# yeyupiaoling/MASR

Measured on NVIDIA H100. Metric: audio_seconds_per_second, higher is better.
Workload: dtype f32 (GEMMs: fp16x2-split operands on wgmma, fp32 accumulate; fp32-grade results)

## Files before the change

masr_b200/csrc/tc_common.cuh:

```cuda
#pragma once
#include <cuda.h>
#include <cuda_fp16.h>
#include <mutex>

#include "common.cuh"

namespace masr {

constexpr float kLoScale = 2048.0f, kLoInv = 1.0f / 2048.0f;

__device__ __forceinline__ uint32_t smem_u32(const void* p) { return (uint32_t)__cvta_generic_to_shared(p); }

__device__ __forceinline__ void mbar_init(uint64_t* bar, uint32_t count) {
    asm volatile("mbarrier.init.shared::cta.b64 [%0], %1;" ::"r"(smem_u32(bar)), "r"(count));
}
__device__ __forceinline__ void mbar_expect_tx(uint64_t* bar, uint32_t bytes) {
    asm volatile("mbarrier.arrive.expect_tx.shared::cta.b64 _, [%0], %1;" ::"r"(smem_u32(bar)), "r"(bytes) : "memory");
}
__device__ __forceinline__ void mbar_wait(uint64_t* bar, uint32_t parity) {
    asm volatile(
        "{\n\t"
        ".reg .pred P1;\n\t"
        "WAIT_LOOP:\n\t"
        "mbarrier.try_wait.parity.shared::cta.b64 P1, [%0], %1;\n\t"
        "@P1 bra DONE;\n\t"
        "bra WAIT_LOOP;\n\t"
        "DONE:\n\t"
        "}" ::"r"(smem_u32(bar)), "r"(parity) : "memory");
}
__device__ __forceinline__ void tma_load_2d(const CUtensorMap* map, uint64_t* bar, void* smem_dst, int c0, int c1) {
    asm volatile(
        "cp.async.bulk.tensor.2d.shared::cluster.global.mbarrier::complete_tx::bytes [%0], [%1, {%3, %4}], [%2];"
        ::"r"(smem_u32(smem_dst)), "l"(map), "r"(smem_u32(bar)), "r"(c0), "r"(c1) : "memory");
}
__device__ __forceinline__ void tma_load_2d_multicast(const CUtensorMap* map, uint64_t* bar, void* smem_dst, int c0, int c1,
                                                      uint16_t cta_mask) {
    asm volatile(
        "cp.async.bulk.tensor.2d.shared::cluster.global.mbarrier::complete_tx::bytes.multicast::cluster"
        " [%0], [%1, {%3, %4}], [%2], %5;"
        ::"r"(smem_u32(smem_dst)), "l"(map), "r"(smem_u32(bar)), "r"(c0), "r"(c1), "h"(cta_mask) : "memory");
}
__device__ __forceinline__ uint32_t cluster_map(uint32_t a, uint32_t rank) {
    uint32_t r;
    asm volatile("mapa.shared::cluster.u32 %0, %1, %2;" : "=r"(r) : "r"(a), "r"(rank));
    return r;
}
__device__ __forceinline__ void cluster_sync() {
    asm volatile("barrier.cluster.arrive.release.aligned;\n\tbarrier.cluster.wait.acquire.aligned;" ::: "memory");
}
__device__ __forceinline__ void tma_prefetch_desc(const CUtensorMap* map) {
    asm volatile("prefetch.tensormap [%0];" ::"l"(map) : "memory");
}
__device__ __forceinline__ bool elect_one_sync() {
    uint32_t pred = 0, laneid = 0;
    asm volatile(
        "{\n\t"
        ".reg .b32 %%rx;\n\t"
        ".reg .pred %%px;\n\t"
        "elect.sync %%rx|%%px, %2;\n\t"
        "@%%px mov.s32 %1, 1;\n\t"
        "mov.s32 %0, %%rx;\n\t"
        "}"
        : "+r"(laneid), "+r"(pred)
        : "r"(0xFFFFFFFFu));
    return pred != 0;
}

__device__ __forceinline__ void wgmma_fence() { asm volatile("wgmma.fence.sync.aligned;" ::: "memory"); }
__device__ __forceinline__ void wgmma_commit() { asm volatile("wgmma.commit_group.sync.aligned;" ::: "memory"); }
template <int N>
__device__ __forceinline__ void wgmma_wait() { asm volatile("wgmma.wait_group.sync.aligned %0;" ::"n"(N) : "memory"); }
template <int R>
__device__ __forceinline__ void reg_fence(float (&d)[R]) {
#pragma unroll
    for (int i = 0; i < R; ++i) asm volatile("" : "+f"(d[i])::"memory");
}
__device__ __forceinline__ void wgmma_m64n128k16_ss(float (&d)[64], uint64_t da, uint64_t db, uint32_t scale_d) {
    asm volatile(
        "{\n\t"
        ".reg .pred p;\n\t"
        "setp.ne.b32 p, %66, 0;\n\t"
        "wgmma.mma_async.sync.aligned.m64n128k16.f32.f16.f16 "
        "{%0, %1, %2, %3, %4, %5, %6, %7, %8, %9, %10, %11, %12, %13, %14, %15, "
        "%16, %17, %18, %19, %20, %21, %22, %23, %24, %25, %26, %27, %28, %29, %30, %31, "
        "%32, %33, %34, %35, %36, %37, %38, %39, %40, %41, %42, %43, %44, %45, %46, %47, "
        "%48, %49, %50, %51, %52, %53, %54, %55, %56, %57, %58, %59, %60, %61, %62, %63}, %64, %65, p, 1, 1, 0, 0;\n\t"
        "}"
        : "+f"(d[0]), "+f"(d[1]), "+f"(d[2]), "+f"(d[3]), "+f"(d[4]), "+f"(d[5]), "+f"(d[6]), "+f"(d[7]), "+f"(d[8]),
          "+f"(d[9]), "+f"(d[10]), "+f"(d[11]), "+f"(d[12]), "+f"(d[13]), "+f"(d[14]), "+f"(d[15]), "+f"(d[16]),
          "+f"(d[17]), "+f"(d[18]), "+f"(d[19]), "+f"(d[20]), "+f"(d[21]), "+f"(d[22]), "+f"(d[23]), "+f"(d[24]),
          "+f"(d[25]), "+f"(d[26]), "+f"(d[27]), "+f"(d[28]), "+f"(d[29]), "+f"(d[30]), "+f"(d[31]), "+f"(d[32]),
          "+f"(d[33]), "+f"(d[34]), "+f"(d[35]), "+f"(d[36]), "+f"(d[37]), "+f"(d[38]), "+f"(d[39]), "+f"(d[40]),
          "+f"(d[41]), "+f"(d[42]), "+f"(d[43]), "+f"(d[44]), "+f"(d[45]), "+f"(d[46]), "+f"(d[47]), "+f"(d[48]),
          "+f"(d[49]), "+f"(d[50]), "+f"(d[51]), "+f"(d[52]), "+f"(d[53]), "+f"(d[54]), "+f"(d[55]), "+f"(d[56]),
          "+f"(d[57]), "+f"(d[58]), "+f"(d[59]), "+f"(d[60]), "+f"(d[61]), "+f"(d[62]), "+f"(d[63])
        : "l"(da), "l"(db), "r"(scale_d));
}
template <int R>
__device__ __forceinline__ void setmaxnreg_inc() { asm volatile("setmaxnreg.inc.sync.aligned.u32 %0;" ::"n"(R)); }
template <int R>
__device__ __forceinline__ void setmaxnreg_dec() { asm volatile("setmaxnreg.dec.sync.aligned.u32 %0;" ::"n"(R)); }

__device__ __forceinline__ uint64_t gmma_desc_sw64(uint32_t smem_addr) {
    uint64_t d = 0;
    d |= (uint64_t)((smem_addr & 0x3FFFF) >> 4);
    d |= (uint64_t)1 << 16;
    d |= (uint64_t)(512 >> 4) << 32;
    d |= (uint64_t)2 << 62;
    return d;
}

__device__ __forceinline__ void add2(float& d0, float& d1, float a0, float a1, float b0, float b1) { d0 = a0 + b0; d1 = a1 + b1; }
__device__ __forceinline__ void sub2(float& d0, float& d1, float a0, float a1, float b0, float b1) { d0 = a0 - b0; d1 = a1 - b1; }
__device__ __forceinline__ void mul2(float& d0, float& d1, float a0, float a1, float b0, float b1) { d0 = a0 * b0; d1 = a1 * b1; }
__device__ __forceinline__ void split_f16(float x, __half& h, __half& l) {
    h = __float2half_rn(x);
    l = __float2half_rn((x - __half2float(h)) * kLoScale);
}
__device__ __forceinline__ void split_f16x2(float x0, float x1, __half2& h, __half2& l) {
    h = __floats2half2_rn(x0, x1);
    const float2 hf = __half22float2(h);
    float d0, d1;
    sub2(d0, d1, x0, x1, hf.x, hf.y);
    mul2(d0, d1, d0, d1, kLoScale, kLoScale);
    l = __floats2half2_rn(d0, d1);
}

__device__ __forceinline__ void mbar_arrive(uint64_t* bar) {
    asm volatile("mbarrier.arrive.shared::cta.b64 _, [%0];" ::"r"(smem_u32(bar)) : "memory");
}
__device__ __forceinline__ void mbar_arrive_cluster(uint32_t a, uint32_t pred) {
    asm volatile("{\n\t.reg .pred p;\n\tsetp.ne.u32 p, %1, 0;\n\t@p mbarrier.arrive.shared::cluster.b64 _, [%0];\n\t}"
                 ::"r"(a), "r"(pred) : "memory");
}

__device__ __forceinline__ void sts128(uint32_t a, const uint4& v) {
    asm volatile("st.shared.v4.b32 [%0], {%1, %2, %3, %4};" ::"r"(a), "r"(v.x), "r"(v.y), "r"(v.z), "r"(v.w) : "memory");
}
__device__ __forceinline__ uint4 lds128(uint32_t a) {
    uint4 v;
    asm volatile("ld.shared.v4.b32 {%0, %1, %2, %3}, [%4];" : "=r"(v.x), "=r"(v.y), "=r"(v.z), "=r"(v.w) : "r"(a) : "memory");
    return v;
}

typedef CUresult (*EncodeTiledFn)(CUtensorMap*, CUtensorMapDataType, cuuint32_t, void*, const cuuint64_t*, const cuuint64_t*,
                                  const cuuint32_t*, const cuuint32_t*, CUtensorMapInterleave, CUtensorMapSwizzle,
                                  CUtensorMapL2promotion, CUtensorMapFloatOOBfill);

inline EncodeTiledFn get_encode_fn() {
    static EncodeTiledFn fn = nullptr;
    static std::once_flag once;
    std::call_once(once, [] {
        void* p = nullptr;
        cudaDriverEntryPointQueryResult qres;
        if (cudaGetDriverEntryPoint("cuTensorMapEncodeTiled", &p, cudaEnableDefault, &qres) == cudaSuccess &&
            qres == cudaDriverEntryPointSuccess)
            fn = reinterpret_cast<EncodeTiledFn>(p);
    });
    return fn;
}

}
```

masr_b200/csrc/tc_gemm.cu:

```cuda
#include <cuda.h>
#include <cuda_fp16.h>
#include <math.h>
#include <mutex>
#include <stdlib.h>
#include <string.h>

#include "tc_common.cuh"

namespace masr {

constexpr int TBM = 128, TBN = 128, TBK = 32;
constexpr int TILE_BYTES = TBM * TBK * 2;
constexpr int STAGE_BYTES = 4 * TILE_BYTES;
constexpr int EW = 8;
constexpr int kStages = 5;
constexpr int RES_BYTES = TBM * TBN * 4;
constexpr int TC_THREADS = 32 * EW + 128;
constexpr int PRODUCER_REGS = 40, CONSUMER_REGS = 232;
static_assert(PRODUCER_REGS * 128 + CONSUMER_REGS * 32 * EW <= 65536, "register file of the SM");

struct TcParams {
    const float* bias;
    const float* residual;
    float* C;
    __half* Ch;
    __half* Cl;
    int64_t ldr, ldc;
    int M, N, K;
    int epi;
    float alpha;
    int conv_T2;
    int flags;
    float* part_m;
    float* part_s;
    int* part_i;
};

constexpr int EPI_CTC_PARTIAL = 8;

struct TcMaps {
    CUtensorMap a[8];
    CUtensorMap w[2];
};

constexpr int CHUNK_KB = 256 / TBK;
constexpr int CONV_TR = 6, CONV_W2 = 19, CONV_ROWS = CONV_TR * CONV_W2;

__device__ __forceinline__ void tma_load_4d(const CUtensorMap* map, uint64_t* bar, void* smem_dst, int c0, int c1, int c2, int c3) {
    asm volatile(
        "cp.async.bulk.tensor.4d.shared::cluster.global.mbarrier::complete_tx::bytes [%0], [%1, {%3, %4, %5, %6}], [%2];"
        ::"r"(smem_u32(smem_dst)), "l"(map), "r"(smem_u32(bar)), "r"(c0), "r"(c1), "r"(c2), "r"(c3) : "memory");
}

struct EpiCtx {
    uint32_t sb;
    int lane;
    int64_t row0;
    int nvalid;
};

template <int CH>
__device__ __forceinline__ void staged_store(const EpiCtx& c, const uint4 (&regs)[CH], uint8_t* g0, int64_t pitch_bytes) {
    constexpr int RSH = (CH == 8) ? 0 : (CH == 4) ? 1 : 2;
    constexpr int RPI = 32 / CH;
    __syncwarp();
#pragma unroll
    for (int k = 0; k < CH; ++k) sts128(c.sb + c.lane * (CH * 16) + ((k ^ ((c.lane >> RSH) & (CH - 1))) << 4), regs[k]);
    __syncwarp();
    const int sub = c.lane / CH, k = c.lane % CH;
    uint4 v[CH];
#pragma unroll
    for (int i = 0; i < CH; ++i) {
        const int row = i * RPI + sub;
        v[i] = lds128(c.sb + row * (CH * 16) + ((k ^ ((row >> RSH) & (CH - 1))) << 4));
    }
#pragma unroll
    for (int i = 0; i < CH; ++i) {
        const int row = i * RPI + sub;
        if (row < c.nvalid) *reinterpret_cast<uint4*>(g0 + row * pitch_bytes + (k << 4)) = v[i];
    }
}

__device__ __forceinline__ void staged_load(const EpiCtx& c, uint4 (&regs)[8], const uint8_t* g0, int64_t pitch_bytes) {
    __syncwarp();
    const int sub = c.lane >> 3, k = c.lane & 7;
    uint4 v[8];
#pragma unroll
    for (int i = 0; i < 8; ++i) {
        const int row = i * 4 + sub;
        v[i] = make_uint4(0, 0, 0, 0);
        if (row < c.nvalid) v[i] = *reinterpret_cast<const uint4*>(g0 + row * pitch_bytes + (k << 4));
    }
#pragma unroll
    for (int i = 0; i < 8; ++i) {
        const int row = i * 4 + sub;
        sts128(c.sb + row * 128 + ((k ^ (row & 7)) << 4), v[i]);
    }
    __syncwarp();
#pragma unroll
    for (int k2 = 0; k2 < 8; ++k2) regs[k2] = lds128(c.sb + c.lane * 128 + ((k2 ^ (c.lane & 7)) << 4));
}

template <int W, int STG>
__device__ __forceinline__ void emit_f32(const EpiCtx& c, float* C, int64_t ld, int flags, const float (&o)[W], int n, int n_limit) {
    const bool full = n + W - 1 < n_limit;
    const bool row_ok = c.lane < c.nvalid;
    const int64_t my_row = c.row0 + c.lane;
    if ((flags & 1) && full && (ld & 3) == 0 && (reinterpret_cast<uintptr_t>(C) & 15) == 0) {
        constexpr int CH = (W / 4 < STG / 512) ? W / 4 : STG / 512;
#pragma unroll
        for (int part = 0; part < (W / 4) / CH; ++part) {
            uint4 regs[CH];
#pragma unroll
            for (int j = 0; j < CH; ++j) {
                const int e = (part * CH + j) * 4;
                regs[j] = make_uint4(__float_as_uint(o[e]), __float_as_uint(o[e + 1]), __float_as_uint(o[e + 2]), __float_as_uint(o[e + 3]));
            }
            staged_store<CH>(c, regs, reinterpret_cast<uint8_t*>(C + c.row0 * ld + n + part * CH * 4), ld * 4);
        }
    } else if (row_ok && full && (ld & 3) == 0 && (reinterpret_cast<uintptr_t>(C) & 15) == 0) {
        float* cp = C + my_row * ld + n;
#pragma unroll
        for (int j = 0; j < W; j += 4) *reinterpret_cast<float4*>(cp + j) = make_float4(o[j], o[j + 1], o[j + 2], o[j + 3]);
    } else if (row_ok) {
        float* cp = C + my_row * ld + n;
#pragma unroll
        for (int j = 0; j < W; ++j)
            if (n + j < n_limit) cp[j] = o[j];
    }
}

template <int W, int STG>
__device__ __forceinline__ void emit_pair(const EpiCtx& c, __half* Ch, __half* Cl, int64_t ld, int flags, const float (&o)[W], int n,
                                          int n_limit) {
    const bool full = n + W - 1 < n_limit;
    const bool row_ok = c.lane < c.nvalid;
    const int64_t my_row = c.row0 + c.lane;
    uint32_t hh[W / 2], ll[W / 2];
#pragma unroll
    for (int j = 0; j < W / 2; ++j) {
        __half2 h2, l2;
        split_f16x2(o[2 * j], o[2 * j + 1], h2, l2);
        hh[j] = *reinterpret_cast<uint32_t*>(&h2);
        ll[j] = *reinterpret_cast<uint32_t*>(&l2);
    }
    const bool aligned = (ld & 7) == 0 && ((reinterpret_cast<uintptr_t>(Ch) | reinterpret_cast<uintptr_t>(Cl)) & 15) == 0;
    if ((flags & 1) && full && aligned) {
        constexpr int CH = (W / 8 < STG / 512) ? W / 8 : STG / 512;
#pragma unroll
        for (int part = 0; part < (W / 8) / CH; ++part) {
            uint4 regs[CH];
#pragma unroll
            for (int j = 0; j < CH; ++j) { const int e = 4 * (part * CH + j); regs[j] = make_uint4(hh[e], hh[e + 1], hh[e + 2], hh[e + 3]); }
            staged_store<CH>(c, regs, reinterpret_cast<uint8_t*>(Ch + c.row0 * ld + n + part * CH * 8), ld * 2);
#pragma unroll
            for (int j = 0; j < CH; ++j) { const int e = 4 * (part * CH + j); regs[j] = make_uint4(ll[e], ll[e + 1], ll[e + 2], ll[e + 3]); }
            staged_store<CH>(c, regs, reinterpret_cast<uint8_t*>(Cl + c.row0 * ld + n + part * CH * 8), ld * 2);
        }
    } else if (row_ok && full && aligned) {
        uint4* hp = reinterpret_cast<uint4*>(Ch + my_row * ld + n);
        uint4* lp = reinterpret_cast<uint4*>(Cl + my_row * ld + n);
#pragma unroll
        for (int j = 0; j < W / 8; ++j) {
            hp[j] = make_uint4(hh[4 * j], hh[4 * j + 1], hh[4 * j + 2], hh[4 * j + 3]);
            lp[j] = make_uint4(ll[4 * j], ll[4 * j + 1], ll[4 * j + 2], ll[4 * j + 3]);
        }
    } else if (row_ok) {
        unsigned short* hp = reinterpret_cast<unsigned short*>(Ch + my_row * ld + n);
        unsigned short* lp = reinterpret_cast<unsigned short*>(Cl + my_row * ld + n);
#pragma unroll
        for (int j = 0; j < W / 2; ++j) {
            if (n + 2 * j < n_limit) { hp[2 * j] = (unsigned short)(hh[j] & 0xffff); lp[2 * j] = (unsigned short)(ll[j] & 0xffff); }
            if (n + 2 * j + 1 < n_limit) { hp[2 * j + 1] = (unsigned short)(hh[j] >> 16); lp[2 * j + 1] = (unsigned short)(ll[j] >> 16); }
        }
    }
}

template <int W, int STG>
__device__ __forceinline__ void emit(const TcParams& p, const EpiCtx& c, const float (&o)[W], int n, int n_limit) {
    if (p.C) emit_f32<W, STG>(c, p.C, p.ldc, p.flags, o, n, n_limit);
    if (p.Ch) emit_pair<W, STG>(c, p.Ch, p.Cl, p.ldc, p.flags, o, n, n_limit);
}

template <int STG>
__device__ __forceinline__ void store_chunk(const TcParams& p, const EpiCtx& c, float (&v)[32], int n) {
    constexpr bool BIG = STG >= 4096;
    if (p.epi == EPI_CTC_PARTIAL) {
        if (n + 31 >= p.N) {
#pragma unroll
            for (int j = 0; j < 32; ++j)
                if (n + j >= p.N) v[j] = -INFINITY;
        }
        float m = v[0];
#pragma unroll
        for (int j = 1; j < 32; ++j) m = fmaxf(m, v[j]);
        int mj = 31;
#pragma unroll
        for (int j = 30; j >= 0; --j)
            if (v[j] == m) mj = j;
        const int mi = n + mj;
        const float mneg = -m * 1.4426950408889634f;
        float sum = 0.f;
#pragma unroll
        for (int j = 0; j < 32; ++j) sum += ex2_approx(fmaf(v[j], 1.4426950408889634f, mneg));
        if (c.lane < c.nvalid) {
            const int64_t idx = (int64_t)(n >> 5) * p.M + c.row0 + c.lane;
            p.part_m[idx] = m; p.part_s[idx] = sum; p.part_i[idx] = mi;
        }
        return;
    }
    if (p.epi == MASR_EPI_BIAS_GLU) {
        float o[16];
#pragma unroll
        for (int j = 0; j < 16; j += 8) {
            float e[8];
#pragma unroll
            for (int k = 0; k < 8; ++k) e[k] = ex2_approx(v[2 * (j + k) + 1] * -1.4426950408889634f);
#pragma unroll
            for (int k = 0; k < 8; ++k) e[k] = rcp_approx(1.0f + e[k]);
#pragma unroll
            for (int k = 0; k < 8; ++k) o[j + k] = v[2 * (j + k)] * e[k];
        }
        emit<16, STG>(p, c, o, n >> 1, p.N >> 1);
        return;
    }
    switch (p.epi) {
        case MASR_EPI_BIAS_SILU:
#pragma unroll
            for (int j = 0; j < 32; j += 8) {
                float e[8];
#pragma unroll
                for (int k = 0; k < 8; k += 2) mul2(e[k], e[k + 1], v[j + k], v[j + k + 1], -1.4426950408889634f, -1.4426950408889634f);
#pragma unroll
                for (int k = 0; k < 8; ++k) e[k] = ex2_approx(e[k]);
#pragma unroll
                for (int k = 0; k < 8; k += 2) add2(e[k], e[k + 1], e[k], e[k + 1], 1.0f, 1.0f);
#pragma unroll
                for (int k = 0; k < 8; ++k) e[k] = rcp_approx(e[k]);
#pragma unroll
                for (int k = 0; k < 8; k += 2) mul2(v[j + k], v[j + k + 1], v[j + k], v[j + k + 1], e[k], e[k + 1]);
            }
            break;
        case MASR_EPI_BIAS_RELU:
#pragma unroll
            for (int j = 0; j < 32; ++j) v[j] = v[j] != v[j] ? v[j] : fmaxf(v[j], 0.f);
            break;
        case MASR_EPI_BIAS_SCALE:
#pragma unroll
            for (int j = 0; j < 32; ++j) v[j] *= p.alpha;
            break;
        case MASR_EPI_RESIDUAL: {
            const bool vec_r = (p.ldr & 3) == 0 && (reinterpret_cast<uintptr_t>(p.residual) & 15) == 0;
            if (BIG && (p.flags & 2) && n + 31 < p.N && vec_r) {
                uint4 rr[8];
                staged_load(c, rr, reinterpret_cast<const uint8_t*>(p.residual + c.row0 * p.ldr + n), p.ldr * 4);
#pragma unroll
                for (int j = 0; j < 8; ++j) {
                    v[4 * j] = __uint_as_float(rr[j].x) + p.alpha * v[4 * j];
                    v[4 * j + 1] = __uint_as_float(rr[j].y) + p.alpha * v[4 * j + 1];
                    v[4 * j + 2] = __uint_as_float(rr[j].z) + p.alpha * v[4 * j + 2];
                    v[4 * j + 3] = __uint_as_float(rr[j].w) + p.alpha * v[4 * j + 3];
                }
            } else if (c.lane < c.nvalid && n + 31 < p.N && vec_r) {
                const float* r = p.residual + (c.row0 + c.lane) * p.ldr + n;
#pragma unroll
                for (int j = 0; j < 32; j += 4) {
                    const float4 rv = *reinterpret_cast<const float4*>(r + j);
                    v[j] = rv.x + p.alpha * v[j]; v[j + 1] = rv.y + p.alpha * v[j + 1];
                    v[j + 2] = rv.z + p.alpha * v[j + 2]; v[j + 3] = rv.w + p.alpha * v[j + 3];
                }
            } else if (c.lane < c.nvalid) {
                const float* r = p.residual + (c.row0 + c.lane) * p.ldr + n;
#pragma unroll
                for (int j = 0; j < 32; ++j)
                    if (n + j < p.N) v[j] = r[j] + p.alpha * v[j];
            }
            break;
        }
        default: break;
    }
    emit<32, STG>(p, c, v, n, p.N);
}

constexpr int EPI_STG = 4096;

__device__ __forceinline__ uint32_t res_off(int r, int c) { return (uint32_t)(r * 128 + ((((c >> 2) ^ (r & 7))) << 4) + (c & 3) * 4); }

template <bool CONV>
__global__ void __launch_bounds__(TC_THREADS, 1)
tc_gemm_kernel(const __grid_constant__ TcMaps maps, const __grid_constant__ TcParams p, int num_tiles, int tiles_n, int tiles_t) {
    extern __shared__ uint8_t smem_raw[];
    uint8_t* smem = reinterpret_cast<uint8_t*>((reinterpret_cast<uintptr_t>(smem_raw) + 1023) & ~uintptr_t(1023));
    uint8_t* res = smem + kStages * STAGE_BYTES;
    uint64_t* full_bar = reinterpret_cast<uint64_t*>(res + RES_BYTES);
    uint64_t* empty_bar = full_bar + kStages;

    const int warp = threadIdx.x >> 5, lane = threadIdx.x & 31;
    const int nkb = p.K / TBK;

    if (warp == EW && lane == 0) {
        tma_prefetch_desc(&maps.a[0]); tma_prefetch_desc(&maps.a[1]); tma_prefetch_desc(&maps.w[0]); tma_prefetch_desc(&maps.w[1]);
        for (int s = 0; s < kStages; ++s) { mbar_init(&full_bar[s], 1); mbar_init(&empty_bar[s], EW); }
        asm volatile("fence.mbarrier_init.release.cluster;" ::: "memory");
    }
    __syncthreads();
    pdl_wait();
    pdl_launch_dependents();

    auto decode = [&](int tile, int& n0, int& m0, int& t0, int& b) {
        const int nt = tile % tiles_n;
        const int rest = tile / tiles_n;
        n0 = nt * TBN;
        if (CONV) { t0 = (rest % tiles_t) * CONV_TR; b = rest / tiles_t; m0 = 0; }
        else { m0 = rest * TBM; t0 = 0; b = 0; }
    };

    if (warp >= EW) {
        setmaxnreg_dec<PRODUCER_REGS>();
        if (warp == EW && elect_one_sync()) {
            constexpr uint32_t a_bytes = CONV ? CONV_ROWS * TBK * 2 : TILE_BYTES;
            constexpr uint32_t tx_bytes = 2 * a_bytes + 2 * TILE_BYTES;
            uint32_t kg = 0;
            const int kb_tap = CONV ? p.N / TBK : 1;
            for (int tile = blockIdx.x; tile < num_tiles; tile += gridDim.x) {
                int n0, m0, t0, b;
                decode(tile, n0, m0, t0, b);
                for (int kb = 0; kb < nkb; ++kb, ++kg) {
                    const uint32_t s = kg % kStages;
                    mbar_wait(&empty_bar[s], ((kg / kStages) & 1) ^ 1);
                    uint8_t* st = smem + s * STAGE_BYTES;
                    if (p.flags & 32) {
                        mbar_arrive(&full_bar[s]);
                        continue;
                    }
                    mbar_expect_tx(&full_bar[s], tx_bytes);
                    if (CONV) {
                        const int tap = kb / kb_tap, cj = kb - tap * kb_tap;
                        const int kh = tap / 3, kw = tap - kh * 3;
                        const int plane = (kh & 1) * 2 + (kw & 1);
                        tma_load_4d(&maps.a[2 * plane], &full_bar[s], st, cj * TBK, kw >> 1, t0 + (kh >> 1), b);
                        tma_load_4d(&maps.a[2 * plane + 1], &full_bar[s], st + TILE_BYTES, cj * TBK, kw >> 1, t0 + (kh >> 1), b);
                    } else {
                        tma_load_2d(&maps.a[0], &full_bar[s], st, kb * TBK, m0);
                        tma_load_2d(&maps.a[1], &full_bar[s], st + TILE_BYTES, kb * TBK, m0);
                    }
                    tma_load_2d(&maps.w[0], &full_bar[s], st + 2 * TILE_BYTES, kb * TBK, n0);
                    tma_load_2d(&maps.w[1], &full_bar[s], st + 3 * TILE_BYTES, kb * TBK, n0);
                }
            }
        }
        __syncwarp();
    } else {
        setmaxnreg_inc<CONSUMER_REGS>();
        const int wg = warp >> 2, wi = warp & 3;
        uint8_t* wg_res = res + wg * (RES_BYTES / 2);
        const int nchunks = (nkb + CHUNK_KB - 1) / CHUNK_KB;
        EpiCtx ctx;
        ctx.lane = lane;
        auto map_rows = [&](int m0, int t0, int b, int q) {
            if (CONV) {
                const int rows = min(CONV_ROWS, (p.conv_T2 - t0) * CONV_W2);
                ctx.row0 = ((int64_t)b * p.conv_T2 + t0) * CONV_W2 + q * 32;
                ctx.nvalid = max(0, min(32, rows - q * 32));
            } else {
                ctx.row0 = (int64_t)m0 + q * 32;
                ctx.nvalid = max(0, min(32, p.M - (m0 + q * 32)));
            }
        };
        const uint32_t wg_bar = 1 + wg;
        const uint32_t is_lane0 = lane == 0;
        auto release = [&](uint32_t s) {
            asm volatile("{\n\t.reg .pred p;\n\tsetp.ne.u32 p, %1, 0;\n\t@p mbarrier.arrive.shared::cta.b64 _, [%0];\n\t}"
                         ::"r"(smem_u32(&empty_bar[s])), "r"(is_lane0) : "memory");
        };
        uint32_t kg = 0;
        for (int tile = blockIdx.x; tile < num_tiles; tile += gridDim.x) {
            int n0, m0, t0, b;
            decode(tile, n0, m0, t0, b);
            const int nw = n0 + wi * 32;
            if (p.bias != nullptr && nw + lane < p.N) asm volatile("prefetch.global.L1 [%0];" ::"l"(p.bias + nw + lane));
            float acc[64], cor[64];
            auto frag_addr = [&](int i, int hh) {
                const int R = 16 * wi + (lane >> 2) + 8 * hh, C = 8 * i + 2 * (lane & 3);
                return smem_u32(wg_res) + ((R >> 5) * 4 + (C >> 5)) * EPI_STG + res_off(R & 31, C & 31);
            };
            asm volatile("bar.sync %0, 128;" ::"r"(wg_bar) : "memory");
            if (p.flags & 64) {
                for (int kb = 0; kb < nkb; ++kb, ++kg) {
                    const uint32_t s = kg % kStages;
                    mbar_wait(&full_bar[s], (kg / kStages) & 1);
                    release(s);
                }
            } else for (int c = 0; c < nchunks; ++c) {
                const int kb_end = min(nkb, (c + 1) * CHUNK_KB);
                int pend = -1;
                for (int kb = c * CHUNK_KB; kb < kb_end; ++kb, ++kg) {
                    const uint32_t s = kg % kStages;
                    mbar_wait(&full_bar[s], (kg / kStages) & 1);
                    const uint32_t sa = smem_u32(smem + s * STAGE_BYTES);
                    const uint32_t sa_m = sa + wg * (TILE_BYTES / 2), sw = sa + 2 * TILE_BYTES;
                    const uint64_t dAh = gmma_desc_sw64(sa_m), dAl = gmma_desc_sw64(sa_m + TILE_BYTES);
                    const uint64_t dWh = gmma_desc_sw64(sw), dWl = gmma_desc_sw64(sw + TILE_BYTES);
                    reg_fence(acc); reg_fence(cor);
                    wgmma_fence();
#pragma unroll
                    for (int ks = 0; ks < TBK / 16; ++ks) {
                        const uint64_t adv = (uint64_t)(ks * 2);
                        wgmma_m64n128k16_ss(acc, dAh + adv, dWh + adv, (kb == c * CHUNK_KB && ks == 0) ? 0u : 1u);
                        wgmma_m64n128k16_ss(cor, dAh + adv, dWl + adv, (kb | ks) ? 1u : 0u);
                        wgmma_m64n128k16_ss(cor, dAl + adv, dWh + adv, 1u);
                    }
                    wgmma_commit();
                    wgmma_wait<1>();
                    reg_fence(acc); reg_fence(cor);
                    if (pend >= 0) release((uint32_t)pend);
                    pend = (int)s;
                }
                wgmma_wait<0>();
                reg_fence(acc); reg_fence(cor);
                if (pend >= 0) release((uint32_t)pend);
                if (c + 1 < nchunks) {
#pragma unroll
                    for (int i = 0; i < 16; ++i)
#pragma unroll
                        for (int hh = 0; hh < 2; ++hh) {
                            float x0 = acc[4 * i + 2 * hh], x1 = acc[4 * i + 2 * hh + 1];
                            const uint32_t a = frag_addr(i, hh);
                            if (c > 0) {
                                float s0, s1;
                                asm volatile("ld.shared.v2.f32 {%0, %1}, [%2];" : "=f"(s0), "=f"(s1) : "r"(a) : "memory");
                                x0 = s0 + x0; x1 = s1 + x1;
                            }
                            asm volatile("st.shared.v2.f32 [%0], {%1, %2};" ::"r"(a), "f"(x0), "f"(x1) : "memory");
                        }
                }
            }
#pragma unroll
            for (int i = 0; i < 16; ++i)
#pragma unroll
                for (int hh = 0; hh < 2; ++hh) {
                    const uint32_t a = frag_addr(i, hh);
                    float x0 = acc[4 * i + 2 * hh], x1 = acc[4 * i + 2 * hh + 1];
                    if (nchunks > 1) {
                        float s0, s1;
                        asm volatile("ld.shared.v2.f32 {%0, %1}, [%2];" : "=f"(s0), "=f"(s1) : "r"(a) : "memory");
                        x0 = s0 + x0; x1 = s1 + x1;
                    }
                    x0 = fmaf(cor[4 * i + 2 * hh], kLoInv, x0);
                    x1 = fmaf(cor[4 * i + 2 * hh + 1], kLoInv, x1);
                    asm volatile("st.shared.v2.f32 [%0], {%1, %2};" ::"r"(a), "f"(x0), "f"(x1) : "memory");
                }
            asm volatile("bar.sync %0, 128;" ::"r"(wg_bar) : "memory");
            for (int h = 0; h < 2; ++h) {
                const int q = 2 * wg + h;
                map_rows(m0, t0, b, q);
                ctx.sb = smem_u32(wg_res) + (h * 4 + wi) * EPI_STG;
                if (nw >= p.N) continue;
                float v[32];
#pragma unroll
                for (int k = 0; k < 8; ++k) {
                    const uint4 r4 = lds128(ctx.sb + lane * 128 + ((k ^ (lane & 7)) << 4));
                    v[4 * k] = __uint_as_float(r4.x); v[4 * k + 1] = __uint_as_float(r4.y);
                    v[4 * k + 2] = __uint_as_float(r4.z); v[4 * k + 3] = __uint_as_float(r4.w);
                }
                if (p.bias != nullptr && nw + 31 < p.N && (reinterpret_cast<uintptr_t>(p.bias + nw) & 15) == 0) {
#pragma unroll
                    for (int j = 0; j < 32; j += 4) {
                        const float4 bb = ldg_f4(p.bias + nw + j);
                        v[j] += bb.x; v[j + 1] += bb.y; v[j + 2] += bb.z; v[j + 3] += bb.w;
                    }
                } else if (p.bias != nullptr) {
#pragma unroll
                    for (int j = 0; j < 32; ++j)
                        if (nw + j < p.N) v[j] += __ldg(p.bias + nw + j);
                }
                store_chunk<EPI_STG>(p, ctx, v, nw);
            }
        }
    }
    __syncthreads();
}

constexpr size_t kTcSmem = kStages * STAGE_BYTES + RES_BYTES + 1024 + 256;
static_assert(kTcSmem <= 232448, "tc_gemm shared memory exceeds the 227 KB per-CTA limit of sm_90");

__global__ void __launch_bounds__(256) split_f16_kernel(const float* __restrict__ x, __half* __restrict__ h,
                                                        __half* __restrict__ l, int64_t n) {
    int64_t i = ((int64_t)blockIdx.x * 256 + threadIdx.x) * 4;
    if (i + 3 < n) {
        float4 v = ldg_f4(x + i);
        __half hh[4], ll[4];
        split_f16(v.x, hh[0], ll[0]); split_f16(v.y, hh[1], ll[1]); split_f16(v.z, hh[2], ll[2]); split_f16(v.w, hh[3], ll[3]);
        *reinterpret_cast<uint2*>(h + i) = *reinterpret_cast<const uint2*>(hh);
        *reinterpret_cast<uint2*>(l + i) = *reinterpret_cast<const uint2*>(ll);
    } else {
        for (; i < n; ++i) split_f16(x[i], h[i], l[i]);
    }
}

__global__ void __launch_bounds__(128) ctc_partial_combine_kernel(const float* __restrict__ pm, const float* __restrict__ ps,
                                                                  const int* __restrict__ pi, int M, int groups,
                                                                  int* __restrict__ ids, float* __restrict__ maxp) {
    pdl_wait();
    pdl_launch_dependents();
    const int lane = threadIdx.x & 31, w = threadIdx.x >> 5;
    const int row = blockIdx.x * 32 + lane;
    float m = -INFINITY, s = 0.f;
    int mi = 0x7fffffff;
    if (row < M) {
#pragma unroll 8
        for (int g = w; g < groups; g += 4) {
            const int64_t idx = (int64_t)g * M + row;
            const float gm = __ldg(pm + idx), gs = __ldg(ps + idx);
            const int gi = __ldg(pi + idx);
            if (gm > m) { s = s * expf(m - gm) + gs; m = gm; mi = gi; }
            else s += gs * expf(gm - m);
        }
    }
    __shared__ float sm_[4][32], ss_[4][32];
    __shared__ int si_[4][32];
    sm_[w][lane] = m; ss_[w][lane] = s; si_[w][lane] = mi;
    __syncthreads();
    if (w == 0 && row < M) {
#pragma unroll
        for (int k = 1; k < 4; ++k) {
            const float gm = sm_[k][lane], gs = ss_[k][lane];
            const int gi = si_[k][lane];
            if (gm > m || (gm == m && gi < mi)) { s = s * expf(m - gm) + gs; m = gm; mi = gi; }
            else s += gs * expf(gm - m);
        }
        ids[row] = s == s ? mi : 0;
        maxp[row] = 1.0f / s;
    }
}

static int make_map_2d(CUtensorMap* map, const void* ptr, int64_t rows, int64_t K, int64_t ld) {
    EncodeTiledFn fn = get_encode_fn();
    if (!fn) { set_last_error("cuTensorMapEncodeTiled entry point unavailable"); return MASR_ERR_INTERNAL; }
    cuuint64_t dims[2] = {(cuuint64_t)K, (cuuint64_t)rows};
    cuuint64_t strides[1] = {(cuuint64_t)ld * 2};
    cuuint32_t box[2] = {(cuuint32_t)TBK, (cuuint32_t)TBM};
    cuuint32_t estr[2] = {1, 1};
    CUresult r = fn(map, CU_TENSOR_MAP_DATA_TYPE_FLOAT16, 2, const_cast<void*>(ptr), dims, strides, box, estr,
                    CU_TENSOR_MAP_INTERLEAVE_NONE, CU_TENSOR_MAP_SWIZZLE_64B, CU_TENSOR_MAP_L2_PROMOTION_L2_128B,
                    CU_TENSOR_MAP_FLOAT_OOB_FILL_NONE);
    if (r != CUDA_SUCCESS) { set_last_error("cuTensorMapEncodeTiled failed (%d) rows=%lld K=%lld ld=%lld", (int)r, (long long)rows, (long long)K, (long long)ld); return MASR_ERR_INTERNAL; }
    return MASR_OK;
}

static bool g_tc_attr_set[64] = {false};

static int make_map_plane(CUtensorMap* map, const void* ptr, int B, int TH, int C) {
    EncodeTiledFn fn = get_encode_fn();
    if (!fn) { set_last_error("cuTensorMapEncodeTiled entry point unavailable"); return MASR_ERR_INTERNAL; }
    cuuint64_t dims[4] = {(cuuint64_t)C, 20, (cuuint64_t)TH, (cuuint64_t)B};
    cuuint64_t strides[3] = {(cuuint64_t)C * 2, (cuuint64_t)20 * C * 2, (cuuint64_t)TH * 20 * C * 2};
    cuuint32_t box[4] = {(cuuint32_t)TBK, (cuuint32_t)CONV_W2, (cuuint32_t)CONV_TR, 1};
    cuuint32_t estr[4] = {1, 1, 1, 1};
    CUresult r = fn(map, CU_TENSOR_MAP_DATA_TYPE_FLOAT16, 4, const_cast<void*>(ptr), dims, strides, box, estr,
                    CU_TENSOR_MAP_INTERLEAVE_NONE, CU_TENSOR_MAP_SWIZZLE_64B, CU_TENSOR_MAP_L2_PROMOTION_L2_128B,
                    CU_TENSOR_MAP_FLOAT_OOB_FILL_NONE);
    if (r != CUDA_SUCCESS) { set_last_error("cuTensorMapEncodeTiled(plane) failed (%d) B=%d TH=%d", (int)r, B, TH); return MASR_ERR_INTERNAL; }
    return MASR_OK;
}

static int tc_flags() {
    const char* e = getenv("MASR_TC_FLAGS");
    return e ? atoi(e) : 1;
}

static int num_sms() {
    static int n[64] = {0};
    int dev = 0;
    cudaGetDevice(&dev);
    if (dev < 0 || dev >= 64) dev = 0;
    if (n[dev] == 0) {
        int v = 0;
        if (cudaDeviceGetAttribute(&v, cudaDevAttrMultiProcessorCount, dev) != cudaSuccess || v <= 0) v = 132;
        n[dev] = v;
    }
    return n[dev];
}

static int ensure_tc_attrs() {
    int dev = 0;
    cudaGetDevice(&dev);
    if (dev < 0 || dev >= 64) dev = 0;
    if (!g_tc_attr_set[dev]) {
        cudaError_t e = cudaFuncSetAttribute(tc_gemm_kernel<false>, cudaFuncAttributeMaxDynamicSharedMemorySize, (int)kTcSmem);
        if (e == cudaSuccess) e = cudaFuncSetAttribute(tc_gemm_kernel<true>, cudaFuncAttributeMaxDynamicSharedMemorySize, (int)kTcSmem);
        if (e != cudaSuccess) { set_last_error("tc_gemm smem attr: %s", cudaGetErrorString(e)); return (int)e; }
        g_tc_attr_set[dev] = true;
    }
    return MASR_OK;
}

template <bool CONV>
static void launch_tc(const TcMaps& maps, const TcParams& p, int tiles_n, int tiles_m, int batch, cudaStream_t stream) {
    const int num_tiles = tiles_n * tiles_m * batch;
    const int grid = num_tiles < num_sms() ? num_tiles : num_sms();
    launch_pdl(tc_gemm_kernel<CONV>, dim3(grid), dim3(TC_THREADS), kTcSmem, stream, maps, p, num_tiles, tiles_n, tiles_m);
}

}

using namespace masr;

extern "C" int masr_conv2_tc_f16x2(const void* c1h, const void* c1l, const void* Wh, const void* Wl, const float* bias,
                                   float* out, void* outh, void* outl, int B, int F1, int T2, int C, void* stream) {
    if (B == 0 || T2 == 0) return MASR_OK;
    MASR_REQUIRE(c1h && c1l && Wh && Wl && (out || (outh && outl)), "masr_conv2_tc_f16x2: null pointer");
    MASR_REQUIRE(C == 256 || C == 512, "masr_conv2_tc_f16x2: C=%d unsupported (this build: 256/512)", C);
    const int TH = (F1 + 1) / 2;
    TcMaps maps;
    memset(&maps, 0, sizeof(maps));
    int rc;
    const int64_t plane_elems = (int64_t)B * TH * 20 * C;
    for (int pl = 0; pl < 4; ++pl) {
        if ((rc = make_map_plane(&maps.a[2 * pl], (const __half*)c1h + pl * plane_elems, B, TH, C))) return rc;
        if ((rc = make_map_plane(&maps.a[2 * pl + 1], (const __half*)c1l + pl * plane_elems, B, TH, C))) return rc;
    }
    if ((rc = make_map_2d(&maps.w[0], Wh, C, 9 * C, 9 * C))) return rc;
    if ((rc = make_map_2d(&maps.w[1], Wl, C, 9 * C, 9 * C))) return rc;
    if ((rc = ensure_tc_attrs())) return rc;
    TcParams p{bias, nullptr, out, (__half*)outh, (__half*)outl, 0, C, B * T2 * CONV_W2, C, 9 * C, MASR_EPI_BIAS_RELU, 1.f, T2, tc_flags()};
    const int tiles_n = (C + TBN - 1) / TBN, tiles_t = (T2 + CONV_TR - 1) / CONV_TR;
    launch_tc<true>(maps, p, tiles_n, tiles_t, B, (cudaStream_t)stream);
    return check_launch("tc_gemm_kernel<conv>");
}

extern "C" int masr_split_f16(const float* x, void* h, void* l, int64_t n, void* stream) {
    if (n == 0) return MASR_OK;
    MASR_REQUIRE(x && h && l, "masr_split_f16: null pointer");
    MASR_REQUIRE((reinterpret_cast<uintptr_t>(x) & 15) == 0 && (reinterpret_cast<uintptr_t>(h) & 7) == 0 &&
                 (reinterpret_cast<uintptr_t>(l) & 7) == 0, "masr_split_f16: misaligned pointer");
    int64_t blocks = (n + 1023) / 1024;
    split_f16_kernel<<<(unsigned)blocks, 256, 0, (cudaStream_t)stream>>>(x, (__half*)h, (__half*)l, n);
    return check_launch("split_f16_kernel");
}

extern "C" int masr_gemm_tc_f16x2(const void* Ah, const void* Al, int64_t lda, const void* Wh, const void* Wl,
                                  const float* bias, const float* residual, int64_t ldr, float* C, void* Ch, void* Cl,
                                  int64_t ldc, int M, int N, int K, int epilogue, float alpha, void* stream) {
    if (M == 0 || N == 0) return MASR_OK;
    MASR_REQUIRE(Ah && Al && Wh && Wl, "masr_gemm_tc_f16x2: null operand");
    MASR_REQUIRE(C || (Ch && Cl), "masr_gemm_tc_f16x2: no output");
    MASR_REQUIRE((Ch == nullptr) == (Cl == nullptr), "masr_gemm_tc_f16x2: Ch/Cl must come as a pair");
    MASR_REQUIRE(K > 0 && K % TBK == 0, "masr_gemm_tc_f16x2: K=%d must be a positive multiple of %d", K, TBK);
    MASR_REQUIRE(lda % 8 == 0, "masr_gemm_tc_f16x2: lda=%lld must be a multiple of 8", (long long)lda);
    MASR_REQUIRE(epilogue >= MASR_EPI_BIAS && epilogue <= MASR_EPI_RESIDUAL, "masr_gemm_tc_f16x2: bad epilogue %d", epilogue);
    MASR_REQUIRE(epilogue != MASR_EPI_RESIDUAL || residual, "masr_gemm_tc_f16x2: residual epilogue needs a residual");
    MASR_REQUIRE(epilogue != MASR_EPI_BIAS_GLU || N % 32 == 0, "masr_gemm_tc_f16x2: GLU epilogue needs N %% 32 == 0");
    MASR_REQUIRE(ldc % 8 == 0 || (C && !Ch && ldc % 4 == 0), "masr_gemm_tc_f16x2: ldc=%lld alignment", (long long)ldc);
    TcMaps maps;
    memset(&maps, 0, sizeof(maps));
    int rc;
    if ((rc = make_map_2d(&maps.a[0], Ah, M, K, lda))) return rc;
    if ((rc = make_map_2d(&maps.a[1], Al, M, K, lda))) return rc;
    if ((rc = make_map_2d(&maps.w[0], Wh, N, K, K))) return rc;
    if ((rc = make_map_2d(&maps.w[1], Wl, N, K, K))) return rc;
    if ((rc = ensure_tc_attrs())) return rc;
    TcParams p{bias, residual, C, (__half*)Ch, (__half*)Cl, ldr, ldc, M, N, K, epilogue, alpha, 0, tc_flags()};
    const int tiles_n = (N + TBN - 1) / TBN, tiles_m = (M + TBM - 1) / TBM;
    launch_tc<false>(maps, p, tiles_n, tiles_m, 1, (cudaStream_t)stream);
    return check_launch("tc_gemm_kernel");
}

extern "C" int masr_ctc_head_argmax_tc_f16x2(const void* Ah, const void* Al, int64_t lda, const void* Wh, const void* Wl,
                                             const float* bias, int M, int V, int K, void* workspace, int64_t workspace_bytes,
                                             int* ids, float* maxp, void* stream) {
    if (M == 0) return MASR_OK;
    MASR_REQUIRE(Ah && Al && Wh && Wl && workspace && ids && maxp, "masr_ctc_head_argmax_tc_f16x2: null pointer");
    MASR_REQUIRE(V > 0 && K > 0 && K % TBK == 0 && lda % 8 == 0, "masr_ctc_head_argmax_tc_f16x2: V=%d K=%d lda=%lld", V, K, (long long)lda);
    const int groups = (V + 31) / 32;
    const int64_t need = (int64_t)3 * groups * M * 4;
    MASR_REQUIRE(workspace_bytes >= need, "masr_ctc_head_argmax_tc_f16x2: workspace %lld < %lld bytes", (long long)workspace_bytes, (long long)need);
    TcMaps maps;
    memset(&maps, 0, sizeof(maps));
    int rc;
    if ((rc = make_map_2d(&maps.a[0], Ah, M, K, lda))) return rc;
    if ((rc = make_map_2d(&maps.a[1], Al, M, K, lda))) return rc;
    if ((rc = make_map_2d(&maps.w[0], Wh, V, K, K))) return rc;
    if ((rc = make_map_2d(&maps.w[1], Wl, V, K, K))) return rc;
    if ((rc = ensure_tc_attrs())) return rc;
    TcParams p{bias, nullptr, nullptr, nullptr, nullptr, 0, 0, M, V, K, EPI_CTC_PARTIAL, 1.f, 0, tc_flags()};
    p.part_m = (float*)workspace;
    p.part_s = p.part_m + (int64_t)groups * M;
    p.part_i = (int*)(p.part_s + (int64_t)groups * M);
    const int tiles_n = (V + TBN - 1) / TBN, tiles_m = (M + TBM - 1) / TBM;
    launch_tc<false>(maps, p, tiles_n, tiles_m, 1, (cudaStream_t)stream);
    if ((rc = check_launch("tc_gemm_kernel<ctc>"))) return rc;
    launch_pdl(ctc_partial_combine_kernel, dim3((M + 31) / 32), dim3(128), 0, (cudaStream_t)stream, (const float*)p.part_m,
               (const float*)p.part_s, (const int*)p.part_i, M, groups, ids, maxp);
    return check_launch("ctc_partial_combine_kernel");
}
```

Before: 54540.

## Keep cross-chunk sums in registers and split epilogue staging per warp pair

```diff
diff --git a/masr_b200/csrc/tc_common.cuh b/masr_b200/csrc/tc_common.cuh
--- a/masr_b200/csrc/tc_common.cuh
+++ b/masr_b200/csrc/tc_common.cuh
@@ -96,6 +96,25 @@
           "+f"(d[57]), "+f"(d[58]), "+f"(d[59]), "+f"(d[60]), "+f"(d[61]), "+f"(d[62]), "+f"(d[63])
         : "l"(da), "l"(db), "r"(scale_d));
 }
+__device__ __forceinline__ void wgmma_m64n128k16_ss_zero(float (&d)[64], uint64_t da, uint64_t db) {
+    asm volatile(
+        "{\n\t"
+        "wgmma.mma_async.sync.aligned.m64n128k16.f32.f16.f16 "
+        "{%0, %1, %2, %3, %4, %5, %6, %7, %8, %9, %10, %11, %12, %13, %14, %15, "
+        "%16, %17, %18, %19, %20, %21, %22, %23, %24, %25, %26, %27, %28, %29, %30, %31, "
+        "%32, %33, %34, %35, %36, %37, %38, %39, %40, %41, %42, %43, %44, %45, %46, %47, "
+        "%48, %49, %50, %51, %52, %53, %54, %55, %56, %57, %58, %59, %60, %61, %62, %63}, %64, %65, 0, 1, 1, 0, 0;\n\t"
+        "}"
+        : "=f"(d[0]), "=f"(d[1]), "=f"(d[2]), "=f"(d[3]), "=f"(d[4]), "=f"(d[5]), "=f"(d[6]), "=f"(d[7]), "=f"(d[8]),
+          "=f"(d[9]), "=f"(d[10]), "=f"(d[11]), "=f"(d[12]), "=f"(d[13]), "=f"(d[14]), "=f"(d[15]), "=f"(d[16]),
+          "=f"(d[17]), "=f"(d[18]), "=f"(d[19]), "=f"(d[20]), "=f"(d[21]), "=f"(d[22]), "=f"(d[23]), "=f"(d[24]),
+          "=f"(d[25]), "=f"(d[26]), "=f"(d[27]), "=f"(d[28]), "=f"(d[29]), "=f"(d[30]), "=f"(d[31]), "=f"(d[32]),
+          "=f"(d[33]), "=f"(d[34]), "=f"(d[35]), "=f"(d[36]), "=f"(d[37]), "=f"(d[38]), "=f"(d[39]), "=f"(d[40]),
+          "=f"(d[41]), "=f"(d[42]), "=f"(d[43]), "=f"(d[44]), "=f"(d[45]), "=f"(d[46]), "=f"(d[47]), "=f"(d[48]),
+          "=f"(d[49]), "=f"(d[50]), "=f"(d[51]), "=f"(d[52]), "=f"(d[53]), "=f"(d[54]), "=f"(d[55]), "=f"(d[56]),
+          "=f"(d[57]), "=f"(d[58]), "=f"(d[59]), "=f"(d[60]), "=f"(d[61]), "=f"(d[62]), "=f"(d[63])
+        : "l"(da), "l"(db));
+}
 template <int R>
 __device__ __forceinline__ void setmaxnreg_inc() { asm volatile("setmaxnreg.inc.sync.aligned.u32 %0;" ::"n"(R)); }
 template <int R>
diff --git a/masr_b200/csrc/tc_gemm.cu b/masr_b200/csrc/tc_gemm.cu
--- a/masr_b200/csrc/tc_gemm.cu
+++ b/masr_b200/csrc/tc_gemm.cu
@@ -2,6 +2,7 @@
 #include <cuda_fp16.h>
 #include <math.h>
 #include <mutex>
+#include <type_traits>
 #include <stdlib.h>
 #include <string.h>
 
@@ -14,7 +15,6 @@
 constexpr int STAGE_BYTES = 4 * TILE_BYTES;
 constexpr int EW = 8;
 constexpr int kStages = 5;
-constexpr int RES_BYTES = TBM * TBN * 4;
 constexpr int TC_THREADS = 32 * EW + 128;
 constexpr int PRODUCER_REGS = 40, CONSUMER_REGS = 232;
 static_assert(PRODUCER_REGS * 128 + CONSUMER_REGS * 32 * EW <= 65536, "register file of the SM");
@@ -291,8 +291,8 @@
 tc_gemm_kernel(const __grid_constant__ TcMaps maps, const __grid_constant__ TcParams p, int num_tiles, int tiles_n, int tiles_t) {
     extern __shared__ uint8_t smem_raw[];
     uint8_t* smem = reinterpret_cast<uint8_t*>((reinterpret_cast<uintptr_t>(smem_raw) + 1023) & ~uintptr_t(1023));
-    uint8_t* res = smem + kStages * STAGE_BYTES;
-    uint64_t* full_bar = reinterpret_cast<uint64_t*>(res + RES_BYTES);
+    uint8_t* staging = smem + kStages * STAGE_BYTES;
+    uint64_t* full_bar = reinterpret_cast<uint64_t*>(staging + 2 * EW * EPI_STG);
     uint64_t* empty_bar = full_bar + kStages;
 
     const int warp = threadIdx.x >> 5, lane = threadIdx.x & 31;
@@ -353,21 +353,24 @@
     } else {
         setmaxnreg_inc<CONSUMER_REGS>();
         const int wg = warp >> 2, wi = warp & 3;
-        uint8_t* wg_res = res + wg * (RES_BYTES / 2);
         const int nchunks = (nkb + CHUNK_KB - 1) / CHUNK_KB;
         EpiCtx ctx;
         ctx.lane = lane;
-        auto map_rows = [&](int m0, int t0, int b, int q) {
+        const int pr = wi >> 1, pw = wi & 1;
+        const uint32_t sb_pair = smem_u32(staging + (2 * wg + pr) * 4 * EPI_STG);
+        const uint32_t pair_bar = 1 + 2 * wg + pr;
+        auto pair_sync = [&]() { asm volatile("bar.sync %0, 64;" ::"r"(pair_bar) : "memory"); };
+        const int wr = 64 * wg + 32 * pr;
+        auto map_rows = [&](int m0, int t0, int b) {
             if (CONV) {
                 const int rows = min(CONV_ROWS, (p.conv_T2 - t0) * CONV_W2);
-                ctx.row0 = ((int64_t)b * p.conv_T2 + t0) * CONV_W2 + q * 32;
-                ctx.nvalid = max(0, min(32, rows - q * 32));
+                ctx.row0 = ((int64_t)b * p.conv_T2 + t0) * CONV_W2 + wr;
+                ctx.nvalid = max(0, min(32, rows - wr));
             } else {
-                ctx.row0 = (int64_t)m0 + q * 32;
-                ctx.nvalid = max(0, min(32, p.M - (m0 + q * 32)));
+                ctx.row0 = (int64_t)m0 + wr;
+                ctx.nvalid = max(0, min(32, p.M - (m0 + wr)));
             }
         };
-        const uint32_t wg_bar = 1 + wg;
         const uint32_t is_lane0 = lane == 0;
         auto release = [&](uint32_t s) {
             asm volatile("{\n\t.reg .pred p;\n\tsetp.ne.u32 p, %1, 0;\n\t@p mbarrier.arrive.shared::cta.b64 _, [%0];\n\t}"
@@ -375,87 +378,89 @@
         };
         uint32_t kg = 0;
         for (int tile = blockIdx.x; tile < num_tiles; tile += gridDim.x) {
-            int n0, m0, t0, b;
-            decode(tile, n0, m0, t0, b);
-            const int nw = n0 + wi * 32;
-            if (p.bias != nullptr && nw + lane < p.N) asm volatile("prefetch.global.L1 [%0];" ::"l"(p.bias + nw + lane));
-            float acc[64], cor[64];
-            auto frag_addr = [&](int i, int hh) {
-                const int R = 16 * wi + (lane >> 2) + 8 * hh, C = 8 * i + 2 * (lane & 3);
-                return smem_u32(wg_res) + ((R >> 5) * 4 + (C >> 5)) * EPI_STG + res_off(R & 31, C & 31);
+            {
+                const int nb = (tile % tiles_n) * TBN + 4 * lane;
+                if (p.bias != nullptr && nb < p.N) asm volatile("prefetch.global.L1 [%0];" ::"l"(p.bias + nb));
+            }
+            auto stage = [&](int i, int hh, float x0, float x1) {
+                const uint32_t a = sb_pair + (i >> 2) * EPI_STG + res_off(16 * pw + (lane >> 2) + 8 * hh, 8 * (i & 3) + 2 * (lane & 3));
+                asm volatile("st.shared.v2.f32 [%0], {%1, %2};" ::"r"(a), "f"(x0), "f"(x1) : "memory");
             };
-            asm volatile("bar.sync %0, 128;" ::"r"(wg_bar) : "memory");
             if (p.flags & 64) {
                 for (int kb = 0; kb < nkb; ++kb, ++kg) {
                     const uint32_t s = kg % kStages;
                     mbar_wait(&full_bar[s], (kg / kStages) & 1);
                     release(s);
                 }
-            } else for (int c = 0; c < nchunks; ++c) {
-                const int kb_end = min(nkb, (c + 1) * CHUNK_KB);
-                int pend = -1;
-                for (int kb = c * CHUNK_KB; kb < kb_end; ++kb, ++kg) {
-                    const uint32_t s = kg % kStages;
-                    mbar_wait(&full_bar[s], (kg / kStages) & 1);
-                    const uint32_t sa = smem_u32(smem + s * STAGE_BYTES);
-                    const uint32_t sa_m = sa + wg * (TILE_BYTES / 2), sw = sa + 2 * TILE_BYTES;
-                    const uint64_t dAh = gmma_desc_sw64(sa_m), dAl = gmma_desc_sw64(sa_m + TILE_BYTES);
-                    const uint64_t dWh = gmma_desc_sw64(sw), dWl = gmma_desc_sw64(sw + TILE_BYTES);
-                    reg_fence(acc); reg_fence(cor);
-                    wgmma_fence();
-#pragma unroll
-                    for (int ks = 0; ks < TBK / 16; ++ks) {
-                        const uint64_t adv = (uint64_t)(ks * 2);
-                        wgmma_m64n128k16_ss(acc, dAh + adv, dWh + adv, (kb == c * CHUNK_KB && ks == 0) ? 0u : 1u);
-                        wgmma_m64n128k16_ss(cor, dAh + adv, dWl + adv, (kb | ks) ? 1u : 0u);
-                        wgmma_m64n128k16_ss(cor, dAl + adv, dWh + adv, 1u);
-                    }
-                    wgmma_commit();
-                    wgmma_wait<1>();
+                pair_sync();
+#pragma unroll
+                for (int i = 0; i < 16; ++i) { stage(i, 0, 0.f, 0.f); stage(i, 1, 0.f, 0.f); }
+            } else {
+                float acc[64], cor[64], sum[64];
+#pragma unroll
+                for (int j = 0; j < 64; ++j) sum[j] = -0.0f;
+                for (int c = 0; c < nchunks; ++c) {
+                    const int kb_end = min(nkb, (c + 1) * CHUNK_KB);
+                    int pend = -1;
+                    auto kblock = [&](auto first_acc, auto first_cor) {
+                        const uint32_t s = kg % kStages;
+                        mbar_wait(&full_bar[s], (kg / kStages) & 1);
+                        const uint32_t sa = smem_u32(smem + s * STAGE_BYTES);
+                        const uint32_t sa_m = sa + wg * (TILE_BYTES / 2), sw = sa + 2 * TILE_BYTES;
+                        const uint64_t dAh = gmma_desc_sw64(sa_m), dAl = gmma_desc_sw64(sa_m + TILE_BYTES);
+                        const uint64_t dWh = gmma_desc_sw64(sw), dWl = gmma_desc_sw64(sw + TILE_BYTES);
+                        if (!decltype(first_acc)::value) reg_fence(acc);
+                        if (!decltype(first_cor)::value) reg_fence(cor);
+                        wgmma_fence();
+#pragma unroll
+                        for (int ks = 0; ks < TBK / 16; ++ks) {
+                            const uint64_t adv = (uint64_t)(ks * 2);
+                            if (decltype(first_acc)::value && ks == 0) wgmma_m64n128k16_ss_zero(acc, dAh + adv, dWh + adv);
+                            else wgmma_m64n128k16_ss(acc, dAh + adv, dWh + adv, 1u);
+                            if (decltype(first_cor)::value && ks == 0) wgmma_m64n128k16_ss_zero(cor, dAh + adv, dWl + adv);
+                            else wgmma_m64n128k16_ss(cor, dAh + adv, dWl + adv, 1u);
+                            wgmma_m64n128k16_ss(cor, dAl + adv, dWh + adv, 1u);
+                        }
+                        wgmma_commit();
+                        wgmma_wait<1>();
+                        reg_fence(acc); reg_fence(cor);
+                        if (pend >= 0) release((uint32_t)pend);
+                        pend = (int)s;
+                        ++kg;
+                    };
+                    using T_ = std::true_type;
+                    using F_ = std::false_type;
+                    if (c == 0) kblock(T_{}, T_{});
+                    else kblock(T_{}, F_{});
+                    for (int kb = c * CHUNK_KB + 1; kb < kb_end; ++kb) kblock(F_{}, F_{});
+                    wgmma_wait<0>();
                     reg_fence(acc); reg_fence(cor);
                     if (pend >= 0) release((uint32_t)pend);
-                    pend = (int)s;
+                    if (c + 1 < nchunks) {
+#pragma unroll
+                        for (int j = 0; j < 64; ++j) sum[j] = sum[j] + acc[j];
+                    }
                 }
-                wgmma_wait<0>();
-                reg_fence(acc); reg_fence(cor);
-                if (pend >= 0) release((uint32_t)pend);
-                if (c + 1 < nchunks) {
-#pragma unroll
-                    for (int i = 0; i < 16; ++i)
-#pragma unroll
-                        for (int hh = 0; hh < 2; ++hh) {
-                            float x0 = acc[4 * i + 2 * hh], x1 = acc[4 * i + 2 * hh + 1];
-                            const uint32_t a = frag_addr(i, hh);
-                            if (c > 0) {
-                                float s0, s1;
-                                asm volatile("ld.shared.v2.f32 {%0, %1}, [%2];" : "=f"(s0), "=f"(s1) : "r"(a) : "memory");
-                                x0 = s0 + x0; x1 = s1 + x1;
-                            }
-                            asm volatile("st.shared.v2.f32 [%0], {%1, %2};" ::"r"(a), "f"(x0), "f"(x1) : "memory");
-                        }
-                }
+                pair_sync();
+#pragma unroll
+                for (int i = 0; i < 16; ++i)
+#pragma unroll
+                    for (int hh = 0; hh < 2; ++hh) {
+                        const int e = 4 * i + 2 * hh;
+                        float x0 = acc[e], x1 = acc[e + 1];
+                        if (nchunks > 1) { x0 = sum[e] + x0; x1 = sum[e + 1] + x1; }
+                        stage(i, hh, fmaf(cor[e], kLoInv, x0), fmaf(cor[e + 1], kLoInv, x1));
+                    }
             }
-#pragma unroll
-            for (int i = 0; i < 16; ++i)
-#pragma unroll
-                for (int hh = 0; hh < 2; ++hh) {
-                    const uint32_t a = frag_addr(i, hh);
-                    float x0 = acc[4 * i + 2 * hh], x1 = acc[4 * i + 2 * hh + 1];
-                    if (nchunks > 1) {
-                        float s0, s1;
-                        asm volatile("ld.shared.v2.f32 {%0, %1}, [%2];" : "=f"(s0), "=f"(s1) : "r"(a) : "memory");
-                        x0 = s0 + x0; x1 = s1 + x1;
-                    }
-                    x0 = fmaf(cor[4 * i + 2 * hh], kLoInv, x0);
-                    x1 = fmaf(cor[4 * i + 2 * hh + 1], kLoInv, x1);
-                    asm volatile("st.shared.v2.f32 [%0], {%1, %2};" ::"r"(a), "f"(x0), "f"(x1) : "memory");
-                }
-            asm volatile("bar.sync %0, 128;" ::"r"(wg_bar) : "memory");
+            pair_sync();
+            int n0, m0, t0, b;
+            decode(tile, n0, m0, t0, b);
+            map_rows(m0, t0, b);
+            if (ctx.nvalid == 0) continue;
             for (int h = 0; h < 2; ++h) {
-                const int q = 2 * wg + h;
-                map_rows(m0, t0, b, q);
-                ctx.sb = smem_u32(wg_res) + (h * 4 + wi) * EPI_STG;
-                if (nw >= p.N) continue;
+                const int n = n0 + 64 * h + 32 * pw;
+                if (n >= p.N) break;
+                ctx.sb = sb_pair + (2 * h + pw) * EPI_STG;
                 float v[32];
 #pragma unroll
                 for (int k = 0; k < 8; ++k) {
@@ -463,25 +468,25 @@
                     v[4 * k] = __uint_as_float(r4.x); v[4 * k + 1] = __uint_as_float(r4.y);
                     v[4 * k + 2] = __uint_as_float(r4.z); v[4 * k + 3] = __uint_as_float(r4.w);
                 }
-                if (p.bias != nullptr && nw + 31 < p.N && (reinterpret_cast<uintptr_t>(p.bias + nw) & 15) == 0) {
+                if (p.bias != nullptr && n + 31 < p.N && (reinterpret_cast<uintptr_t>(p.bias + n) & 15) == 0) {
 #pragma unroll
                     for (int j = 0; j < 32; j += 4) {
-                        const float4 bb = ldg_f4(p.bias + nw + j);
+                        const float4 bb = ldg_f4(p.bias + n + j);
                         v[j] += bb.x; v[j + 1] += bb.y; v[j + 2] += bb.z; v[j + 3] += bb.w;
                     }
                 } else if (p.bias != nullptr) {
 #pragma unroll
                     for (int j = 0; j < 32; ++j)
-                        if (nw + j < p.N) v[j] += __ldg(p.bias + nw + j);
+                        if (n + j < p.N) v[j] += __ldg(p.bias + n + j);
                 }
-                store_chunk<EPI_STG>(p, ctx, v, nw);
+                store_chunk<EPI_STG>(p, ctx, v, n);
             }
         }
     }
     __syncthreads();
 }
 
-constexpr size_t kTcSmem = kStages * STAGE_BYTES + RES_BYTES + 1024 + 256;
+constexpr size_t kTcSmem = kStages * STAGE_BYTES + 2 * EW * EPI_STG + 1024 + 256;
 static_assert(kTcSmem <= 232448, "tc_gemm shared memory exceeds the 227 KB per-CTA limit of sm_90");
 
 __global__ void __launch_bounds__(256) split_f16_kernel(const float* __restrict__ x, __half* __restrict__ h,
```

Result: faster. 55560, median of 6 (+1.9%).
